# dvl-tum/e-osvos

Measured on AMD Instinct MI355X. Metric: finetune_iters_per_sec, higher is better.
Workload: dtype f32 (f16x3 split); 1 GPU; e-OSVOS-50 fine-tune iteration (BASELINE configs[1]): DeepLabV3+-ResNet50, batch 3, 480x854, BCE, per-neuron-lr SGD; one (sequence, object) per rank; batch=3, height=480, width=854, parallelism=replicas x1

## Files before the change

### e-osvos_amd/_ffi.py

```python
import ctypes
import os

_HERE = os.path.dirname(os.path.abspath(__file__))
LIB_PATH = os.environ.get('EOSVOS_LIB') or os.path.join(_HERE, 'libeosvos.so')

c_float_p = ctypes.c_void_p
_E = ctypes.c_void_p


class View(ctypes.Structure):
    _fields_ = [('p', ctypes.c_void_p), ('ld', ctypes.c_int), ('key', ctypes.c_void_p), ('ldkey', ctypes.c_int)]


class ConvViews(ctypes.Structure):
    _fields_ = ([(n, ctypes.c_int) for n in ('algo', 'B', 'H', 'W', 'Cin', 'Cout', 'k', 'stride', 'dil', 'pad')] +
                [('w_oihw', ctypes.c_void_p), ('scale', ctypes.c_void_p), ('bias', ctypes.c_void_p), ('passes', ctypes.c_int),
                 ('x', View), ('y', View), ('res', View), ('relu', ctypes.c_int), ('y_m8', ctypes.c_void_p),
                 ('g', View), ('gx', View), ('add', View), ('accum', ctypes.c_int), ('mask_c0', ctypes.c_int),
                 ('gx_m8', ctypes.c_void_p), ('dw_oihw', ctypes.c_void_p),
                 ('slot_bits', ctypes.c_uint * 2), ('slot_valid', ctypes.c_int * 2),
                 ('src_slot_bits', ctypes.c_uint * 2), ('src_slot_valid', ctypes.c_int * 2), ('fwd_slices', ctypes.c_int)])


VIEWS_FWD, VIEWS_DGRAD, VIEWS_WGRAD = 1, 2, 4
# ... 59 lines not shown
    'eosvos_bce': (ctypes.c_int, [_E, c_float_p, c_float_p, ctypes.c_int64, c_float_p, c_float_p]),
    'eosvos_backward_step': (ctypes.c_int, [_E, ctypes.c_int]),
    'eosvos_finetune_step': (ctypes.c_int, [_E, c_float_p, c_float_p, ctypes.c_int, ctypes.c_int,
                                            ctypes.POINTER(ctypes.c_float)]),
    'eosvos_keep_grads': (ctypes.c_int, [_E, ctypes.c_int]),
    'eosvos_get_grads': (ctypes.c_int, [_E, c_float_p]),
    'eosvos_infer': (ctypes.c_int, [_E, c_float_p, ctypes.c_int, c_float_p]),
    'eosvos_infer_view': (ctypes.c_int, [_E, c_float_p, ctypes.c_int, ctypes.c_int]),
    'eosvos_tta_accumulate': (ctypes.c_int, [_E, ctypes.c_int, ctypes.c_int, ctypes.c_int, ctypes.c_int, ctypes.c_float, ctypes.c_int,
                                             c_float_p, ctypes.c_int, ctypes.c_int]),
    'eosvos_resize_frames': (ctypes.c_int, [_E, c_float_p] + [ctypes.c_int] * 6 + [c_float_p]),
    'eosvos_merge_labels': (ctypes.c_int, [_E, c_float_p, ctypes.c_int, ctypes.c_int64, ctypes.c_void_p]),
    'eosvos_meta_task_begin': (ctypes.c_int, [_E]),
    'eosvos_meta_grad': (ctypes.c_int, [_E, c_float_p, c_float_p, ctypes.c_int, c_float_p,
                                        ctypes.POINTER(ctypes.c_float)]),
    'eosvos_meta_grad_ex': (ctypes.c_int, [_E, c_float_p, c_float_p, ctypes.c_int, c_float_p,
                                           ctypes.POINTER(ctypes.c_float), ctypes.c_float, ctypes.c_int]),
    'eosvos_radam_step': (ctypes.c_int, [_E, c_float_p, c_float_p, c_float_p, c_float_p, ctypes.c_int64,
                                         ctypes.c_float, ctypes.c_float, ctypes.c_float, ctypes.c_float,
                                         ctypes.c_float, ctypes.c_int, ctypes.c_float, ctypes.c_float]),
    'eosvos_clamp': (ctypes.c_int, [_E, c_float_p, ctypes.c_int64, ctypes.c_float, ctypes.c_float]),
    'eosvos_outer_step': (ctypes.c_int, [_E, c_float_p, c_float_p, c_float_p, c_float_p, ctypes.c_int64, ctypes.c_int, ctypes.c_int,
                                         ctypes.c_float, ctypes.c_float, ctypes.c_float, ctypes.c_float, ctypes.c_float,
                                         ctypes.c_float, ctypes.c_float, ctypes.c_float, ctypes.c_float, ctypes.c_float,
                                         ctypes.c_int, ctypes.c_int64, ctypes.c_int64]),
    'eosvos_alias_state': (ctypes.c_int, [_E, _E]),
    'eosvos_unalias_state': (ctypes.c_int, [_E]),
    'eosvos_set_trainable_from': (ctypes.c_int, [_E, ctypes.c_int]),
    'eosvos_comm_unique_id': (ctypes.c_int, [ctypes.c_void_p]),
    'eosvos_comm_init_rank': (ctypes.c_int, [ctypes.POINTER(ctypes.c_void_p), ctypes.c_int, ctypes.c_void_p, ctypes.c_int, ctypes.c_int]),
    'eosvos_comm_destroy': (ctypes.c_int, [ctypes.c_void_p]),
    'eosvos_allreduce_sum': (ctypes.c_int, [_E, c_float_p, ctypes.c_int64, ctypes.c_void_p]),
    'eosvos_time_hot_kernel': (ctypes.c_int, [_E, ctypes.c_int, ctypes.c_int, ctypes.POINTER(ctypes.c_float),
                                              ctypes.POINTER(ctypes.c_double)]),
    'eosvos_bench_conv': (ctypes.c_int, [_E, ctypes.c_int, ctypes.c_int, ctypes.c_int, ctypes.c_int,
                                         ctypes.POINTER(ctypes.c_float), ctypes.POINTER(ctypes.c_double)]),
    'eosvos_mfma_probe': (ctypes.c_int, [_E, ctypes.c_int, ctypes.POINTER(ctypes.c_float),
                                         ctypes.POINTER(ctypes.c_double)]),
    'eosvos_profile_launches': (ctypes.c_int, [_E, ctypes.c_int]),
    'eosvos_profile_read': (ctypes.c_int, [_E, ctypes.c_int, ctypes.c_char_p, ctypes.POINTER(ctypes.c_int64),
                                           ctypes.POINTER(ctypes.c_double), ctypes.POINTER(ctypes.c_double),
                                           ctypes.POINTER(ctypes.c_int)]),
    'eosvos_debug_tensor': (ctypes.c_int, [_E, ctypes.c_char_p, ctypes.POINTER(ctypes.c_void_p),
                                           ctypes.POINTER(ctypes.c_int64)]),
    'eosvos_test_conv': (ctypes.c_int, [_E, c_float_p, c_float_p, c_float_p, c_float_p, c_float_p,
                                        ctypes.c_int] + [ctypes.c_int] * 9 + [c_float_p]),
    'eosvos_test_conv_bwd': (ctypes.c_int, [_E, c_float_p, c_float_p, c_float_p] + [ctypes.c_int] * 9 +
                             [c_float_p, c_float_p]),
    'eosvos_test_conv_algo': (ctypes.c_int, [_E, ctypes.c_int, c_float_p, c_float_p, c_float_p, c_float_p, c_float_p,
                                             ctypes.c_int] + [ctypes.c_int] * 9 + [c_float_p]),
    'eosvos_test_conv_bwd_algo': (ctypes.c_int, [_E, ctypes.c_int, c_float_p, c_float_p, c_float_p, c_float_p, ctypes.c_void_p] +
                                  [ctypes.c_int] * 9 + [c_float_p, c_float_p]),
    'eosvos_test_conv_views': (ctypes.c_int, [_E, ctypes.POINTER(ConvViews)]),
    'eosvos_test_aspp_dgrad': (ctypes.c_int, [_E, ctypes.c_int, c_float_p, ctypes.c_void_p, c_float_p, ctypes.c_int,
                                              ctypes.POINTER(ctypes.c_int), ctypes.POINTER(ctypes.c_uint),
                                              ctypes.POINTER(ctypes.c_int)]),
    'eosvos_test_groupnorm': (ctypes.c_int, [_E, ctypes.c_int, c_float_p, ctypes.c_int, c_float_p, ctypes.c_int, c_float_p,
                                             c_float_p, c_float_p, ctypes.c_int, ctypes.c_int, ctypes.c_int, ctypes.c_int,
                                             ctypes.c_int, ctypes.c_float, c_float_p, ctypes.c_int, c_float_p, ctypes.c_void_p,
                                             ctypes.c_int]),
    'eosvos_test_maxpool': (ctypes.c_int, [_E, c_float_p] + [ctypes.c_int] * 4 + [c_float_p, ctypes.c_void_p, c_float_p, c_float_p]),
    'eosvos_test_resize': (ctypes.c_int, [_E] + [ctypes.c_int] * 7 + [c_float_p, ctypes.c_int] * 4 + [ctypes.c_void_p, ctypes.c_int]),
    'eosvos_test_aspp_pool': (ctypes.c_int, [_E] + [ctypes.c_int] * 4 + [c_float_p] * 4 + [ctypes.c_int] + [c_float_p] * 3 +
                              [ctypes.c_int, ctypes.c_void_p, ctypes.c_int, c_float_p, ctypes.c_int] + [c_float_p] * 4 +
                              [ctypes.c_int]),
    'eosvos_test_head': (ctypes.c_int, [_E, c_float_p, c_float_p, c_float_p, ctypes.c_int64, ctypes.c_int] + [c_float_p] * 4),
    'eosvos_test_wgrad_presplit': (ctypes.c_int, [c_float_p] * 8 + [ctypes.c_int] * 15 + [ctypes.c_void_p]),
}

_lib = None


class EosvosError(RuntimeError):
    pass


def load():
    global _lib
    if _lib is not None:
        return _lib
    if not os.path.exists(LIB_PATH):
        raise EosvosError(
            f'{LIB_PATH} is missing: build it with `python -c "import __graft_entry__ as g; g.build()"` '
            '(hipcc --offload-arch=gfx950).  There is no CPU fallback.')
    lib = ctypes.CDLL(LIB_PATH)
    for name, (res, args) in _SIGNATURES.items():
        fn = getattr(lib, name)
        fn.restype = res
        fn.argtypes = args
    _lib = lib
    return lib


def exported_symbols():
    return sorted(_SIGNATURES)


def check(rc):
    if rc != 0:
        raise EosvosError(load().eosvos_last_error().decode() or f'eosvos call failed ({rc})')
```

### e-osvos_amd/csrc/engine.cpp

```cpp
#include <dlfcn.h>
#include <hip/hip_runtime.h>
#include <math.h>
#include <stdio.h>
#include <stdlib.h>
#include <string.h>

#include <algorithm>
#include <cmath>
#include <functional>
#include <map>
#include <set>
#include <string>
#include <vector>

#include "../../include/eosvos.h"
#include "kernels.h"

using namespace eosvos;

static thread_local std::string g_err;
static int fail(const std::string& m) {
  g_err = m;
  return 1;
}
// ... 3086 lines not shown
  launch_oihw_to_ohwi(w_oihw, t->Wp, Cout, Cin, k * k, t->s);
  if (scale) {
    HIPOK(hipMemcpyAsync(t->na, scale, (size_t)Cout * 4, hipMemcpyDeviceToDevice, t->s));
    HIPOK(hipMemcpyAsync(t->nb, bias, (size_t)Cout * 4, hipMemcpyDeviceToDevice, t->s));
  }
  if (res && wino_on(t, 0, B, conv_out(H, k, stride, dil, pad), conv_out(W, k, stride, dil, pad)))
    return fail("the Winograd output transform has no residual input (the network never needs one)");
  conv_fwd(t, 0, x, Cin, H, W, y, Cout, B, res, Cout, relu != 0);
  HIPOK(hipStreamSynchronize(t->s));
  HIPOK(hipGetLastError());
  return 0;
}
int eosvos_test_conv_bwd_algo(eosvos_engine* e, int algo, const float* x, const float* w_oihw, const float* g,
                              const float* scale, const uint8_t* m8, int B, int H, int W, int Cin, int Cout, int k, int stride,
                              int dil, int pad, float* dx, float* dw_oihw) {
  ModeScope mode_scope(e);
  if (!e || !x || !w_oihw || !g || !dx || !dw_oihw) return fail("null argument");
  if (Cin % 4 || Cout % 4) return fail("channels must be multiples of 4");
  if (algo < EOSVOS_ALGO_AUTO || algo > EOSVOS_ALGO_WINO_F4) return fail("unknown conv algorithm");
  ScratchEngine se(e, algo, B, H, W, Cin, Cout, k, stride, dil, pad, scale != nullptr);
  if (!se.ok) return fail("scratch engine: shape not eligible for the requested algorithm, or out of memory");
  eosvos_engine* t = &se.t;
  const int T = k * k;
  amax_new_phase(t, 0);
  amax_new_phase(t, 1);
  launch_oihw_to_ohwi(w_oihw, t->Wp, Cout, Cin, T, t->s);
  if (scale) HIPOK(hipMemcpyAsync(t->na, scale, (size_t)Cout * 4, hipMemcpyDeviceToDevice, t->s));
  conv_wgrad(t, 0, g, Cout, x, Cin, H, W, B);
  if (m8) t->mask8[x] = const_cast<uint8_t*>(m8);
  if (conv_dgrad(t, 0, g, Cout, H, W, dx, Cin, B, false, m8 ? x : nullptr, 0)) return 1;
  float* dw = t->falloc((int64_t)Cout * Cin * T);
  if (!dw) return fail("hipMalloc dw");
  const int64_t n = (int64_t)Cout * Cin * T;
  launch_sgd_update(dw, t->ws_wg, t->upd_splits[0], n, scale ? t->na : nullptr, nullptr, nullptr, dw, (int64_t)T * Cin, n, t->s);
  launch_ohwi_to_oihw(dw, dw_oihw, Cout, Cin, T, 1.f, 0, t->s);
  HIPOK(hipStreamSynchronize(t->s));
  HIPOK(hipGetLastError());
  return 0;
}
int eosvos_test_conv(eosvos_engine* e, const float* x, const float* w_oihw, const float* scale, const float* bias,
                     const float* res, int relu, int B, int H, int W, int Cin, int Cout, int k, int stride, int dil,
                     int pad, float* y) {
  ModeScope mode_scope(e);
  return eosvos_test_conv_algo(e, EOSVOS_ALGO_DIRECT, x, w_oihw, scale, bias, res, relu, B, H, W, Cin, Cout, k, stride, dil, pad, y);
}
int eosvos_test_conv_bwd(eosvos_engine* e, const float* x, const float* w_oihw, const float* g, int B, int H, int W,
                         int Cin, int Cout, int k, int stride, int dil, int pad, float* dx, float* dw_oihw) {
  ModeScope mode_scope(e);
  return eosvos_test_conv_bwd_algo(e, EOSVOS_ALGO_DIRECT, x, w_oihw, g, nullptr, nullptr, B, H, W, Cin, Cout, k, stride, dil, pad, dx,
                                   dw_oihw);
}

namespace {
int read_tslot(eosvos_engine* t, int phase, const float* key, unsigned* bits, int* valid) {
  *bits = 0; *valid = 0;
  if (!h3_mode() || !t->amax) return 0;
  auto it = t->treg[phase].find(key);
  if (it == t->treg[phase].end()) return 0;
  unsigned w[AMAX_SUB];
  HIPOK(hipMemcpy2D(w, sizeof(unsigned), t->amax + amax_tcol(t, phase, it->second.idx), (size_t)AMAX_ROW * sizeof(unsigned),
                    sizeof(unsigned), AMAX_SUB, hipMemcpyDeviceToHost));
  for (int i = 0; i < AMAX_SUB; ++i) *bits = w[i] > *bits ? w[i] : *bits;
  *valid = it->second.valid ? 1 : 0;
  return 0;
}
int seed_tslot(eosvos_engine* t, int phase, const float* key, long rows, int C) {
  if (!h3_mode()) return 0;
  if (amax_init(t)) return fail("absmax arena");
  unsigned* sl = tslot(t, phase, key);
  if (!sl) return fail("no absmax slot left for the source tensor");
  launch_absmax(key, rows, C, C, sl, t->s);
  tmark_valid(t, phase, key);
  return 0;
}
bool view_ok(const eosvos_view& v, int C) {
  if (!v.p || v.ld < C || (v.ld & 3)) return false;
  if (!v.key) return true;
  const long off = v.p - v.key;
  return v.ldkey == v.ld && off >= 0 && !(off & 3) && off + C <= v.ldkey;
}
}

int eosvos_test_conv_views(eosvos_engine* e, eosvos_conv_views* v) {
  ModeScope mode_scope(e);
  if (!e || !v || !v->w_oihw) return fail("null argument");
  const int B = v->B, H = v->H, W = v->W, Cin = v->Cin, Cout = v->Cout, k = v->k;
  if (B < 1 || H < 1 || W < 1 || Cin < 4 || Cout < 4 || (Cin % 4) || (Cout % 4)) return fail("bad geometry (channels must be multiples of 4)");
  if (v->algo < EOSVOS_ALGO_AUTO || v->algo > EOSVOS_ALGO_WINO_F4) return fail("unknown conv algorithm");
  const bool fwd = v->passes & EOSVOS_VIEWS_FWD, dg = v->passes & EOSVOS_VIEWS_DGRAD, wg = v->passes & EOSVOS_VIEWS_WGRAD;
  if (!fwd && !dg && !wg) return fail("no pass selected");
  if (fwd && (v->scale == nullptr) != (v->bias == nullptr)) return fail("scale and bias go together (folded norm)");
  if (fwd && (!view_ok(v->x, Cin) || !view_ok(v->y, Cout) || (v->res.p && !view_ok(v->res, Cout)))) return fail("bad forward view");
  const int nsl = v->fwd_slices > 1 ? v->fwd_slices : 1;
  if (nsl > 1) {
    if (!fwd || dg || wg || v->res.p || !v->x.key || !v->y.key) return fail("fwd_slices: forward only, keyed x and y, no residual");
    if ((v->x.p - v->x.key) + (long)nsl * Cin > v->x.ldkey || (v->y.p - v->y.key) + (long)nsl * Cout > v->y.ldkey) return fail("fwd_slices: past the tensor");
  }
  if ((dg || wg) && !view_ok(v->g, Cout)) return fail("bad gradient view");
  if (dg && (!view_ok(v->gx, Cin) || (v->add.p && !view_ok(v->add, Cin)) || v->mask_c0 < 0 || (v->mask_c0 & 3))) return fail("bad data-gradient view");
  if (wg && (!view_ok(v->x, Cin) || !v->dw_oihw)) return fail("bad weight-gradient view");
  ScratchEngine se(e, v->algo, B, H, W, Cin, Cout, k, v->stride, v->dil, v->pad, v->scale != nullptr);
  if (!se.ok) return fail("scratch engine: shape not eligible for the requested algorithm, or out of memory");
  eosvos_engine* t = &se.t;
  const int T = k * k;
  const int Ho = conv_out(H, k, v->stride, v->dil, v->pad), Wo = conv_out(W, k, v->stride, v->dil, v->pad);
  const long Pin = (long)B * H * W, Pout = (long)B * Ho * Wo;
// ... 231 lines not shown
```

### e-osvos_amd/csrc/kernels.h

```cpp
#pragma once
#include <hip/hip_runtime.h>
#include <stdint.h>

namespace eosvos {
#define AMAX_SUB 32
#define AMAX_ROW 2048
#if defined(__HIPCC__)
__device__ __forceinline__ unsigned amax_f1(float x) {
  const unsigned a = __float_as_uint(x) & 0x7fffffffu;
  return a < 0x7f800000u ? a : 0u;
}
__device__ __forceinline__ unsigned amax_f4(unsigned m, const float4& v) {
  const unsigned a = amax_f1(v.x), b = amax_f1(v.y), c = amax_f1(v.z), d = amax_f1(v.w);
  const unsigned ab = a > b ? a : b, cd = c > d ? c : d;
  const unsigned q = ab > cd ? ab : cd;
  return m > q ? m : q;
}
__device__ __forceinline__ uint8_t relu_bits(const float4& v) {
  return (uint8_t)((v.x > 0.f ? 1 : 0) | (v.y > 0.f ? 2 : 0) | (v.z > 0.f ? 4 : 0) | (v.w > 0.f ? 8 : 0));
}
__device__ __forceinline__ void relu_mask8(float4& v, unsigned bits) {
  v.x = (bits & 1u) ? v.x : 0.f; v.y = (bits & 2u) ? v.y : 0.f; v.z = (bits & 4u) ? v.z : 0.f; v.w = (bits & 8u) ? v.w : 0.f;
}
__device__ __forceinline__ void amax_block_commit(unsigned m, unsigned* slot) {
// ... 147 lines not shown
  int B, Ho, Wo, ldg, Cout;
  int Hi, Wi, ldx, Cin;
  int KH, KW, stride, pad, dil;
  int splits;
  long g_tap_stride, x_tap_stride;
  const unsigned* amax_g;
  const unsigned* amax_x;
  float* scn_g; float* scn_x;
  int margin_g, margin_x;
};
void launch_wgrad(const WgradArgs& a, hipStream_t s);
int wgrad_pick_splits(int P, int Cout, int Cin, int T, int wg_budget = 0, int mode = -1);
int wgrad_group_tile(int channels);
void launch_wgrad_group(const WgradArgs* dev_tab, const int* dev_map, int nwg, int bm, int bn, double flops, hipStream_t s);
struct WgradPArgs {
  const unsigned char* g2;
  const unsigned char* x2;
  float* ws;
  int B, Ho, Wo, ldg, Cout;
  int Hi, Wi, ldx, Cin;
  int KH, KW, stride, pad, dil;
  int splits;
  int groups;
  long g_tap_stride, x_tap_stride;
  const unsigned char* zero;
  const float* scp_g; const float* scp_x;
  const unsigned* slot_g; const unsigned* slot_x;
  float* scn_g; float* scn_x;
  int margin_g, margin_x;
  const float* g; const float* x;
};
#define PAIR_HEADROOM 10
bool wgrad_p_supported(const WgradPArgs& a);
int wgrad_p_tiles(const WgradPArgs& a);
void launch_wgrad_p(const WgradPArgs& a, hipStream_t s);
int wgrad_p_pick_splits(int P, int Cout, int Cin, int T, int wg_budget);
int wgrad_p_resident(int wg_budget);
void launch_wgrad_p_group(const WgradPArgs* dev_tab, const int* dev_map, int nwg, double flops, hipStream_t s);
void launch_pair_split(const float* x, void* out, long rows, int C, int ld, const unsigned* slot, int margin, float* sc, hipStream_t s);
int conv_wg_budget_of(int requested);
int conv_clamp_wg_budget(int n);
void launch_wino_input(int tm, const float* x, int ldx, int C, int B, int H, int W, int th, int tw, int dil, long prow, float* V,
                       hipStream_t s, unsigned* amax = nullptr);
void launch_wino_grad(int tm, const float* g, int ldg, int C, int B, int H, int W, int th, int tw, int dil, long prow, float* M,
                      hipStream_t s, unsigned* amax = nullptr);
void launch_wino_weight(int tm, const float* w, int Cout, int Cin, const float* rowscale, float* U, float* Us, hipStream_t s,
                        unsigned* amax_u = nullptr, unsigned* amax_us = nullptr);
void launch_wino_output(int tm, const float* M, long prow, int C, int B, int H, int W, int th, int tw, int dil, const float* scale,
                        const float* bias, int relu, float* y, int ldy, hipStream_t s, unsigned* amax = nullptr,
                        uint8_t* mask8_out = nullptr, int ldm8 = 0);
void launch_wino_wgrad_finish(int tm, const float* ws, int splits, int Cout, int Cin, float* dst, hipStream_t s);
void launch_wino_dgrad_output(int tm, const float* dV, long prow, int C, int B, int H, int W, int th, int tw, int dil,
                              const uint8_t* mask8, int ldm8, int mask_c0, int accum, float* gx, int ldgx, hipStream_t s,
                              unsigned* amax = nullptr);

void launch_nchw_to_nhwc_pad(const float* src, float* dst, int B, int C, int H, int W, int pad,
                             hipStream_t s, unsigned* amax = nullptr, int mirror = 0);
void launch_fill(float* p, int64_t n, float v, hipStream_t s);
void launch_oihw_to_ohwi(const float* src, float* dst, int O, int I, int T, hipStream_t s);
void launch_ohwi_to_oihw(const float* src, float* dst, int O, int I, int T, float alpha, int add,
                         hipStream_t s);
void launch_fold_norm(const float* gamma, const float* beta, const float* mean, const float* var,
                      float eps, float* a, float* b, int64_t n, hipStream_t s);

void launch_stem_fwd(const float* xpad, const float* w , const float* a,
                     const float* b, float* y, int B, int H, int W, int Ho, int Wo, hipStream_t s);
void launch_stem_wgrad(const float* xpad, const float* g, float* ws , int B,
                       int H, int W, int Ho, int Wo, int chunks, hipStream_t s);
int stem_wgrad_chunks(int B, int Ho, int Wo);
void launch_stem_fwd_h3(const float* xpad, const float* w , const float* a, const float* b, float* y, int B,
                        int H, int W, int Ho, int Wo, const unsigned* amax_x, hipStream_t s);
void launch_stem_wgrad_h3(const float* xpad, const float* g, float* ws , int B, int H, int W, int Ho,
                          int Wo, int chunks, const unsigned* amax_g, const unsigned* amax_x, hipStream_t s);

void launch_maxpool_fwd(const float* x, float* y, uint8_t* idx, int B, int H, int W, int C, int Ho,
                        int Wo, hipStream_t s, unsigned* amax = nullptr);
void launch_maxpool_bwd(const float* gy, const uint8_t* idx, float* gx, int B, int H,
                        int W, int C, int Ho, int Wo, hipStream_t s, unsigned* amax = nullptr);

struct ResizeTab {
  int in, out;
  const int* i0;
  const int* i1;
  const float* lam;
  const int* lo;
  const int* hi;
};
void launch_resize_fwd(const float* x, int ldx, float* y, int ldy, int B, int C, ResizeTab th,
                       ResizeTab tw, hipStream_t s);
void launch_resize_bwd(const float* gy, int ldgy, float* gx, int ldgx, const uint8_t* m8, int ldm8,
                       int B, int C, ResizeTab th, ResizeTab tw, hipStream_t s, unsigned* amax = nullptr);

void launch_colsum(const float* x, int ldx, float* out , int B, int P, int C, float alpha,
                   float* scratch, hipStream_t s);
void launch_gemv_fwd(const float* W, const float* v, const float* a, const float* b, float* y, int B,
                     int N, int K, hipStream_t s);
void launch_gemv_bwd(const float* W, const float* v, const float* gp, const float* a, float* gv,
                     float* dW, int B, int N, int K, hipStream_t s);
void launch_bcast_pixels(const float* v , float* y, int ldy, int B, int P, int C, float alpha,
                         hipStream_t s, uint8_t* mask8_out = nullptr, int ldm8 = 0);

void launch_last_fwd(const float* x, const float* w, const float* bias, float* y, int64_t P, int C,
                     hipStream_t s);
void launch_last_bwd(const float* x, const float* w, const float* g, float* gx, float* ws_dw,
                     int64_t P, int C, int chunks, hipStream_t s);
int last_bwd_chunks(int64_t P);

// ... 106 lines not shown
```

### e-osvos_amd/csrc/misc_kernels.hip

```cpp
#include <cassert>

#include "kernels.h"

namespace eosvos {

__device__ __forceinline__ float wave_sum(float v) {
#pragma unroll
  for (int o = 32; o > 0; o >>= 1) v += __shfl_xor(v, o, 64);
  return v;
}
__device__ __forceinline__ float block_sum_256(float v, float* sh ) {
  v = wave_sum(v);
  const int w = threadIdx.x >> 6;
  __syncthreads();
  if ((threadIdx.x & 63) == 0) sh[w] = v;
  __syncthreads();
  return sh[0] + sh[1] + sh[2] + sh[3];
}
static inline int grid_for(long n, int per_block, int cap = 4096) {
  long b = (n + per_block - 1) / per_block;
  if (b < 1) b = 1;
  if (b > cap) b = cap;
  return (int)b;
}
// ... 2058 lines not shown
        const int tx = blk.tx + dl;
        if ((unsigned)tx >= (unsigned)tw) continue;
        const long tile = ((((long)b * dil + sy) * dil + sx) * th + ty) * tw + tx;
#pragma unroll
        for (int ii = 0; ii < 2; ++ii) {
          const int i = dk < 0 ? 3 : (dk > 0 ? 0 : 1 + ii);
          if (dk != 0 && ii == 1) continue;
          const int r = dk < 0 ? 0 : (dk > 0 ? 1 : ii);
#pragma unroll
          for (int jj = 0; jj < 2; ++jj) {
            const int j = dl < 0 ? 3 : (dl > 0 ? 0 : 1 + jj);
            if (dl != 0 && jj == 1) continue;
            const int q = dl < 0 ? 0 : (dl > 0 ? 1 : jj);
            float4 sum = zero4();
#pragma unroll
            for (int a = 0; a < 4; ++a) {
              if (Mt::BT[a][i] == 0.f) continue;
#pragma unroll
              for (int bb = 0; bb < 4; ++bb) {
                if (Mt::BT[bb][j] == 0.f) continue;
                const float4 v = *reinterpret_cast<const float4*>(dV + ((long)(a * 4 + bb) * prow + tile) * C + c4 * 4);
                const float wgt = Mt::BT[a][i] * Mt::BT[bb][j];
                sum.x += wgt * v.x; sum.y += wgt * v.y; sum.z += wgt * v.z; sum.w += wgt * v.w;
              }
            }
            acc[r][q].x += sum.x; acc[r][q].y += sum.y; acc[r][q].z += sum.z; acc[r][q].w += sum.w;
          }
        }
      }
    }
#pragma unroll
    for (int r = 0; r < 2; ++r) {
      const int yy = sy + dil * (2 * blk.ty + r);
      if (yy >= H) continue;
#pragma unroll
      for (int q = 0; q < 2; ++q) {
        const int xx = sx + dil * (2 * blk.tx + q);
        if (xx >= W) continue;
        const long pix = ((long)b * H + yy) * W + xx;
        float4 v = acc[r][q];
        if (accum) {
          const float4 o = *reinterpret_cast<const float4*>(gx + pix * ldgx + c4 * 4);
          v.x += o.x; v.y += o.y; v.z += o.z; v.w += o.w;
        }
        if (mask8 && c4 * 4 >= mask_c0) relu_mask8(v, mask8[pix * ldm8 + c4]);
        am = amax_f4(am, v);
        *reinterpret_cast<float4*>(gx + pix * ldgx + c4 * 4) = v;
      }
    }
  }
  if (amax) amax_block_commit(am, amax);
}

#define WINO_LAUNCH(kernel, grid, s, ...)                                                              \
  do {                                                                                                 \
    assert(tm == 2 || tm == 4);                                                                        \
    if (tm == 4) hipLaunchKernelGGL(kernel<4>, dim3(grid), dim3(256), 0, s, __VA_ARGS__);              \
    else hipLaunchKernelGGL(kernel<2>, dim3(grid), dim3(256), 0, s, __VA_ARGS__);                      \
  } while (0)
void launch_wino_input(int tm, const float* x, int ldx, int C, int B, int H, int W, int th, int tw, int dil, long prow, float* V,
                       hipStream_t s, unsigned* amax) {
  const long n = (long)B * dil * dil * th * tw * (C / 4);
  WINO_LAUNCH(wino_input_kernel, grid_for(n, 256, 8192), s, x, ldx, C, B, H, W, th, tw, dil, prow, V, amax);
}
void launch_wino_grad(int tm, const float* g, int ldg, int C, int B, int H, int W, int th, int tw, int dil, long prow, float* M,
                      hipStream_t s, unsigned* amax) {
  const long n = (long)B * dil * dil * th * tw * (C / 4);
  WINO_LAUNCH(wino_grad_kernel, grid_for(n, 256, 8192), s, g, ldg, C, B, H, W, th, tw, dil, prow, M, amax);
}
void launch_wino_weight(int tm, const float* w, int Cout, int Cin, const float* rowscale, float* U, float* Us, hipStream_t s,
                        unsigned* amax_u, unsigned* amax_us) {
  const long n = (long)Cout * (Cin / 4);
  WINO_LAUNCH(wino_weight_kernel, grid_for(n, 256), s, w, Cout, Cin, rowscale, U, Us, amax_u, amax_us);
}
void launch_wino_output(int tm, const float* M, long prow, int C, int B, int H, int W, int th, int tw, int dil, const float* scale,
                        const float* bias, int relu, float* y, int ldy, hipStream_t s, unsigned* amax, uint8_t* mask8_out, int ldm8) {
  const long n = (long)B * dil * dil * th * tw * (C / 4);
  WINO_LAUNCH(wino_output_kernel, grid_for(n, 256, 8192), s, M, prow, C, B, H, W, th, tw, dil, scale, bias, relu, y, ldy, amax,
              relu ? mask8_out : nullptr, ldm8);
}
void launch_wino_wgrad_finish(int tm, const float* ws, int splits, int Cout, int Cin, float* dst, hipStream_t s) {
  const long n = (long)Cout * (Cin / (tm == 4 ? wino_finish_cin_per_thread<4> : wino_finish_cin_per_thread<2>));
  WINO_LAUNCH(wino_wgrad_finish_kernel, grid_for(n, 256), s, ws, splits, Cout, Cin, dst);
}
void launch_wino_dgrad_output(int tm, const float* dV, long prow, int C, int B, int H, int W, int th, int tw, int dil,
                              const uint8_t* mask8, int ldm8, int mask_c0, int accum, float* gx, int ldgx, hipStream_t s,
                              unsigned* amax) {
  const long n = (long)B * dil * dil * th * tw * (C / 4);
  WINO_LAUNCH(wino_dgrad_output_kernel, grid_for(n, 256, 8192), s, dV, prow, C, B, H, W, th, tw, dil, mask8, ldm8, mask_c0, accum,
              gx, ldgx, amax);
}
#undef WINO_LAUNCH
}
```

### e-osvos_amd/engine.py

```python
import ctypes

import torch

from . import _ffi
from .topology import ARCH_ID, norm_layers, trainable


def _ptr(t):
    return ctypes.c_void_p(t.data_ptr())


def _optr(t):
    return _ptr(t) if t is not None else None


def _relu_bits(t):
    if t is None:
        return None
    m = (t > 0).to(torch.uint8).reshape(*t.shape[:-1], -1, 4)
    return (m[..., 0] | (m[..., 1] << 1) | (m[..., 2] << 2) | (m[..., 3] << 3)).contiguous()


def _ld(t):
    if t is None:
# ... 662 lines not shown
        _ffi.check(self.lib.eosvos_mfma_probe(self.h, iters, ctypes.byref(ms), ctypes.byref(fl)))
        return fl.value / (ms.value * 1e-3) / 1e12

    def debug_tensor(self, name):
        ptr = ctypes.c_void_p()
        dims = (ctypes.c_int64 * 4)()
        _ffi.check(self.lib.eosvos_debug_tensor(self.h, name.encode(), ctypes.byref(ptr), dims))
        b, h, w, c = [int(d) for d in dims]
        n = b * h * w * c
        out = torch.empty(n, device=self.device)
        self.synchronize()
        import ctypes as _c
        hip = _c.CDLL('libamdhip64.so')
        rc = hip.hipMemcpy(_c.c_void_p(out.data_ptr()), ptr, _c.c_size_t(n * 4), 3)
        if rc != 0:
            raise _ffi.EosvosError(f'hipMemcpy failed ({rc})')
        return out.view(b, h, w, c).permute(0, 3, 1, 2).contiguous()

    def test_conv(self, x_nhwc, w_oihw, scale, bias, res, relu, stride, dil, pad):
        B, H, W, Cin = x_nhwc.shape
        Cout, _, k, _ = w_oihw.shape
        Ho = (H + 2 * pad - dil * (k - 1) - 1) // stride + 1
        Wo = (W + 2 * pad - dil * (k - 1) - 1) // stride + 1
        y = torch.empty(B, Ho, Wo, Cout, device=self.device)
        p = lambda t: _ptr(t) if t is not None else None
        _ffi.check(self.lib.eosvos_test_conv(self.h, _ptr(x_nhwc), _ptr(w_oihw), p(scale), p(bias), p(res),
                                             int(relu), B, H, W, Cin, Cout, k, stride, dil, pad, _ptr(y)))
        return y

    ALGOS = {'auto': 0, 'direct': 1, 'wino_f2': 2, 'wino_f4': 3}

    def test_conv_algo(self, algo, x_nhwc, w_oihw, scale, bias, res, relu, stride, dil, pad):
        B, H, W, Cin = x_nhwc.shape
        Cout, _, k, _ = w_oihw.shape
        Ho = (H + 2 * pad - dil * (k - 1) - 1) // stride + 1
        Wo = (W + 2 * pad - dil * (k - 1) - 1) // stride + 1
        y = torch.empty(B, Ho, Wo, Cout, device=self.device)
        p = lambda t: _ptr(t) if t is not None else None
        _ffi.check(self.lib.eosvos_test_conv_algo(self.h, self.ALGOS[algo], _ptr(x_nhwc), _ptr(w_oihw), p(scale), p(bias),
                                                  p(res), int(relu), B, H, W, Cin, Cout, k, stride, dil, pad, _ptr(y)))
        return y

    def test_conv_bwd_algo(self, algo, x_nhwc, w_oihw, g_nhwc, stride, dil, pad, scale=None, mask=None):
        B, H, W, Cin = x_nhwc.shape
        Cout, _, k, _ = w_oihw.shape
        dx = torch.empty_like(x_nhwc)
        dw = torch.empty_like(w_oihw)
        m8 = _relu_bits(mask)
        _ffi.check(self.lib.eosvos_test_conv_bwd_algo(self.h, self.ALGOS[algo], _ptr(x_nhwc), _ptr(w_oihw), _ptr(g_nhwc),
                                                      _optr(scale), _optr(m8), B, H, W, Cin, Cout, k, stride, dil, pad, _ptr(dx),
                                                      _ptr(dw)))
        return dx, dw

    def test_conv_bwd(self, x_nhwc, w_oihw, g_nhwc, stride, dil, pad):
        B, H, W, Cin = x_nhwc.shape
        Cout, _, k, _ = w_oihw.shape
        dx = torch.empty_like(x_nhwc)
        dw = torch.empty_like(w_oihw)
        _ffi.check(self.lib.eosvos_test_conv_bwd(self.h, _ptr(x_nhwc), _ptr(w_oihw), _ptr(g_nhwc), B, H, W, Cin,
                                                 Cout, k, stride, dil, pad, _ptr(dx), _ptr(dw)))
        return dx, dw

    @staticmethod
    def _view(t, C, shape):
        v = _ffi.View()
        if t is None:
            return v
        view, base = t if isinstance(t, tuple) else (t, None)
        B, h, w = shape
        ld = view.stride(2)
        assert view.dtype == torch.float32 and tuple(view.shape) == (B, h, w, C), (tuple(view.shape), (B, h, w, C))
        assert view.stride() == (h * w * ld, w * ld, ld, 1) and ld >= C and ld % 4 == 0, view.stride()
        v.p, v.ld = view.data_ptr(), ld
        if base is None:
            assert view.is_contiguous() or view._base is not None, 'a strided view needs its base tensor'
            if view._base is not None:
                b0 = view._base
                off = (view.data_ptr() - b0.data_ptr()) // 4
                assert 0 <= off and off + (B * h * w - 1) * ld + C <= b0.numel(), 'view outside its storage'
        else:
            assert base.dtype == torch.float32 and base.is_contiguous() and tuple(base.shape) == (B, h, w, ld), tuple(base.shape)
            off = (view.data_ptr() - base.data_ptr()) // 4
            assert 0 <= off <= ld - C and off % 4 == 0, off
            v.key, v.ldkey = base.data_ptr(), ld
        return v

    def test_conv_views(self, algo, w_oihw, stride, dil, pad, shape, scale=None, bias=None, x=None, y=None, res=None, relu=False,
                        y_m8=None, g=None, gx=None, add=None, accum=False, mask_c0=0, gx_m8=None, want_dw=False, fwd_slices=1):
        B, H, W = shape
        Cout, Cin, k, _ = w_oihw.shape
        Ho = (H + 2 * pad - dil * (k - 1) - 1) // stride + 1
        Wo = (W + 2 * pad - dil * (k - 1) - 1) // stride + 1
        a = _ffi.ConvViews()
        a.algo, a.B, a.H, a.W, a.Cin, a.Cout, a.k, a.stride, a.dil, a.pad = self.ALGOS[algo], B, H, W, Cin, Cout, k, stride, dil, pad
        assert w_oihw.is_contiguous() and w_oihw.dtype == torch.float32
        a.w_oihw = w_oihw.data_ptr()
        for name, t in (('scale', scale), ('bias', bias)):
            if t is not None:
                assert t.is_contiguous() and t.dtype == torch.float32 and t.numel() == Cout
                setattr(a, name, t.data_ptr())
        a.passes = (_ffi.VIEWS_FWD if y is not None else 0) | (_ffi.VIEWS_DGRAD if gx is not None else 0) | (_ffi.VIEWS_WGRAD if want_dw else 0)
        a.x, a.y, a.res = self._view(x, Cin, (B, H, W)), self._view(y, Cout, (B, Ho, Wo)), self._view(res, Cout, (B, Ho, Wo))
        a.g, a.gx, a.add = self._view(g, Cout, (B, Ho, Wo)), self._view(gx, Cin, (B, H, W)), self._view(add, Cin, (B, H, W))
        a.relu, a.accum, a.mask_c0, a.fwd_slices = int(relu), int(accum), int(mask_c0), int(fwd_slices)
        if fwd_slices > 1:
            for vw, C in ((a.x, Cin), (a.y, Cout)):
# ... 106 lines not shown
```

### include/eosvos.h

```cpp
#ifndef EOSVOS_H
#define EOSVOS_H

#include <stddef.h>
#include <stdint.h>

#ifdef __cplusplus
extern "C" {
#endif

typedef struct eosvos_engine eosvos_engine;

#define EOSVOS_ARCH_RESNET50 50
#define EOSVOS_ARCH_RESNET101 101
#define EOSVOS_ARCH_V3_RESNET50 1050
#define EOSVOS_ARCH_V3_RESNET101 1101
#define EOSVOS_NORM_BN_FROZEN 0
#define EOSVOS_NORM_GN16 1

const char* eosvos_version(void);
const char* eosvos_last_error(void);

#define EOSVOS_MATRIX_F32 0
#define EOSVOS_MATRIX_BF16X6 1
#define EOSVOS_MATRIX_F16X3 2
// ... 108 lines not shown
                     float* flat_meta_grad, float* meta_loss_host);
#define EOSVOS_META_INIT_GRAD 1
#define EOSVOS_META_NEW_SEGMENT 2
int eosvos_meta_grad_ex(eosvos_engine* e, const float* images, const float* masks, int batch,
                        float* flat_meta_grad, float* meta_loss_host, float weight, int flags);

int eosvos_radam_step(eosvos_engine* e, float* param, const float* grad, float* exp_avg,
                      float* exp_avg_sq, int64_t n, float lr, float weight_decay, float beta1,
                      float beta2, float eps, int step, float grad_scale, float grad_clip);
int eosvos_clamp(eosvos_engine* e, float* param, int64_t n, float lo, float hi);
int eosvos_outer_step(eosvos_engine* e, float* state, float* grad, float* exp_avg, float* exp_avg_sq, int64_t n_lr,
                      int learn_model_init, int step, float lr_lr, float init_lr, float weight_decay, float beta1, float beta2,
                      float eps, float grad_scale, float grad_clip, float lr_lo, float lr_hi, int use_log,
                      int64_t frozen_lr, int64_t frozen_param);
int eosvos_alias_state(eosvos_engine* e, eosvos_engine* src);
int eosvos_unalias_state(eosvos_engine* e);

int eosvos_set_trainable_from(eosvos_engine* e, int conv_idx);

typedef struct { char internal[128]; } eosvos_rccl_id;
int eosvos_comm_unique_id(eosvos_rccl_id* id);
int eosvos_comm_init_rank(void** comm, int world_size, const eosvos_rccl_id* id, int rank, int device_id);
int eosvos_comm_destroy(void* comm);
int eosvos_allreduce_sum(eosvos_engine* e, float* flat, int64_t n, void* comm);

int eosvos_time_hot_kernel(eosvos_engine* e, int batch, int reps, float* ms_host,
                           double* flops_host);
int eosvos_bench_conv(eosvos_engine* e, int conv_idx, int kind, int batch, int reps, float* ms_host,
                      double* flops_host);
int eosvos_mfma_probe(eosvos_engine* e, int iters, float* ms_host, double* flops_host);
int eosvos_profile_launches(eosvos_engine* e, int on);
int eosvos_profile_read(eosvos_engine* e, int max_kernels, char* names, int64_t* counts, double* ms_host,
                        double* flops_host, int* n_out_host);
int eosvos_debug_tensor(eosvos_engine* e, const char* name, float** ptr_out, int64_t* dims4_out);
int eosvos_test_conv(eosvos_engine* e, const float* x_nhwc, const float* w_oihw,
                     const float* scale, const float* bias, const float* res_nhwc, int relu,
                     int B, int H, int W, int Cin, int Cout, int k, int stride, int dil, int pad,
                     float* y_nhwc);
#define EOSVOS_ALGO_AUTO 0
#define EOSVOS_ALGO_DIRECT 1
#define EOSVOS_ALGO_WINO_F2 2
#define EOSVOS_ALGO_WINO_F4 3
int eosvos_test_conv_algo(eosvos_engine* e, int algo, const float* x_nhwc, const float* w_oihw,
                          const float* scale, const float* bias, const float* res_nhwc, int relu,
                          int B, int H, int W, int Cin, int Cout, int k, int stride, int dil, int pad,
                          float* y_nhwc);
int eosvos_test_conv_bwd_algo(eosvos_engine* e, int algo, const float* x_nhwc, const float* w_oihw,
                              const float* g_nhwc, const float* scale, const uint8_t* m8, int B, int H, int W,
                              int Cin, int Cout, int k, int stride, int dil, int pad, float* dx_nhwc,
                              float* dw_oihw);
int eosvos_test_conv_bwd(eosvos_engine* e, const float* x_nhwc, const float* w_oihw,
                         const float* g_nhwc, int B, int H, int W, int Cin, int Cout, int k,
                         int stride, int dil, int pad, float* dx_nhwc, float* dw_oihw);

typedef struct eosvos_view {
  float* p;
  int ld;
  float* key;
  int ldkey;
} eosvos_view;
#define EOSVOS_VIEWS_FWD 1
#define EOSVOS_VIEWS_DGRAD 2
#define EOSVOS_VIEWS_WGRAD 4
typedef struct eosvos_conv_views {
  int algo, B, H, W, Cin, Cout, k, stride, dil, pad;
  const float* w_oihw;
  const float* scale;
  const float* bias;
  int passes;
  eosvos_view x, y, res;
  int relu;
  uint8_t* y_m8;
  eosvos_view g, gx, add;
  int accum, mask_c0;
  const uint8_t* gx_m8;
  float* dw_oihw;
  unsigned slot_bits[2];
  int slot_valid[2];
  unsigned src_slot_bits[2];
  int src_slot_valid[2];
  int fwd_slices;
} eosvos_conv_views;
int eosvos_test_conv_views(eosvos_engine* e, eosvos_conv_views* v);
int eosvos_test_aspp_dgrad(eosvos_engine* e, int batch, const float* g_cat, const uint8_t* l4_m8, float* g_l4_inout,
                           int force_fallback, int* merged_ran, unsigned* slot_bits, int* slot_valid);

int eosvos_test_groupnorm(eosvos_engine* e, int bwd, float* z, int ldz, const float* g, int ldg, const float* gamma,
                          const float* beta, const float* res, int ldres, int relu, int B, int P, int C, float eps, float* y,
                          int ldy, float* stats, uint8_t* m8, int ldm8);
int eosvos_test_maxpool(eosvos_engine* e, const float* x, int B, int H, int W, int C, float* y, uint8_t* idx, const float* gy,
                        float* gx);
int eosvos_test_resize(eosvos_engine* e, int align_corners, int hin, int win, int hout, int wout, int B, int C, const float* x,
                       int ldx, float* y, int ldy, const float* gy, int ldgy, float* gx, int ldgx, const uint8_t* m8, int ldm8);
int eosvos_test_aspp_pool(eosvos_engine* e, int B, int P, int K, int N, const float* w, const float* a, const float* bias,
                          const float* x, int ldx, float* v, float* pool, float* y, int ldy, uint8_t* m8, int ldm8,
                          const float* gy, int ldgy, float* gpool, float* gv, float* dw, float* gx, int ldgx);
int eosvos_test_head(eosvos_engine* e, const float* x, const float* w, const float* bias, int64_t P, int C, float* y,
                     const float* g, float* gx, float* dw);

int eosvos_test_wgrad_presplit(const float* g, const float* x, float* ws, void* g2, void* x2, unsigned* amax, float* sc,
                               const void* zero, int B, int Ho, int Wo, int Cout, int Hi, int Wi, int Cin, int k, int stride,
                               int pad, int dil, int splits, int groups, int margin, int which, void* stream);

#ifdef __cplusplus
}
#endif
// ... 2 lines not shown
```

Baseline: 114.5 finetune_iters/s.

## Share Winograd F4 dgrad output-transform partials between neighbour tiles via LDS

Adds an LDS-based Winograd F(4,3) dgrad output kernel. Each thread handles one tile and channel quad within a 4x4 tile block, computes its own stage-1 transform once, and exchanges edge rows and columns with neighbouring tiles through shared memory, instead of re-reading and re-transforming neighbour dV tiles from global memory. The kernel becomes the default for tm=4, dil=1. Tiles on a block boundary still fall back to global loads. The cost is extra registers (a 6x6 float4 array per thread), several barriers, and a new test entry point to compare the two forms.

New measurement: 115.0 finetune_iters/s, median of 6. No clear change (+0.5%).

```diff
diff --git a/e-osvos_amd/_ffi.py b/e-osvos_amd/_ffi.py
--- a/e-osvos_amd/_ffi.py
+++ b/e-osvos_amd/_ffi.py
@@ -135,6 +135,9 @@
     'eosvos_test_conv_bwd_algo': (ctypes.c_int, [_E, ctypes.c_int, c_float_p, c_float_p, c_float_p, c_float_p, ctypes.c_void_p] +
                                   [ctypes.c_int] * 9 + [c_float_p, c_float_p]),
     'eosvos_test_conv_views': (ctypes.c_int, [_E, ctypes.POINTER(ConvViews)]),
+    'eosvos_test_wino_dgrad_output': (ctypes.c_int, [_E, ctypes.c_int, c_float_p] + [ctypes.c_int] * 4 + [ctypes.c_void_p,
+                                                     ctypes.c_int, ctypes.c_int, c_float_p, ctypes.c_int,
+                                                     ctypes.POINTER(ctypes.c_uint)]),
     'eosvos_test_aspp_dgrad': (ctypes.c_int, [_E, ctypes.c_int, c_float_p, ctypes.c_void_p, c_float_p, ctypes.c_int,
                                               ctypes.POINTER(ctypes.c_int), ctypes.POINTER(ctypes.c_uint),
                                               ctypes.POINTER(ctypes.c_int)]),
diff --git a/e-osvos_amd/csrc/engine.cpp b/e-osvos_amd/csrc/engine.cpp
--- a/e-osvos_amd/csrc/engine.cpp
+++ b/e-osvos_amd/csrc/engine.cpp
@@ -3162,6 +3162,41 @@
 }
 
 namespace {
+struct TestAmaxArena {
+  unsigned* d = nullptr;
+  TestAmaxArena() {
+    if (hipMalloc(&d, (size_t)AMAX_SUB * AMAX_ROW * sizeof(unsigned)) != hipSuccess) d = nullptr;
+    if (d) (void)hipMemset(d, 0, (size_t)AMAX_SUB * AMAX_ROW * sizeof(unsigned));
+  }
+  ~TestAmaxArena() { if (d) (void)hipFree(d); }
+  unsigned* slot(int s) const { return d + s; }
+  int read(int s, unsigned* bits) const {
+    unsigned w[AMAX_SUB];
+    HIPOK(hipMemcpy2D(w, sizeof(unsigned), d + s, (size_t)AMAX_ROW * sizeof(unsigned), sizeof(unsigned), AMAX_SUB, hipMemcpyDeviceToHost));
+    *bits = 0;
+    for (int i = 0; i < AMAX_SUB; ++i) *bits = w[i] > *bits ? w[i] : *bits;
+    return 0;
+  }
+};
+}
+int eosvos_test_wino_dgrad_output(eosvos_engine* e, int form, const float* dV, int B, int H, int W, int C, const uint8_t* m8,
+                                  int mask_c0, int accum, float* gx, int ldgx, unsigned* amax_bits) {
+  if (!e || !dV || !gx || !amax_bits) return fail("null argument");
+  if (form < 0 || form > 1) return fail("form: 0 gather, 1 LDS");
+  if (B < 1 || H < 1 || W < 1 || C < 4 || (C & 3) || ldgx < C || (ldgx & 3) || mask_c0 < 0 || (mask_c0 & 3)) return fail("bad geometry");
+  if (form == 1 && !wino_dgrad_output_lds_ok(4, 1, C)) return fail("the LDS form does not take this shape");
+  const int th = (H + 3) / 4, tw = (W + 3) / 4;
+  const long ntile = (long)B * th * tw;
+  TestAmaxArena am;
+  if (!am.d) return fail("hipMalloc absmax arena");
+  launch_wino_dgrad_output(4, dV, ntile, C, B, H, W, th, tw, 1, m8, ldgx / 4, mask_c0, accum ? 1 : 0, gx, ldgx, e->s, am.slot(0),
+                           form == 0);
+  HIPOK(hipStreamSynchronize(e->s));
+  HIPOK(hipGetLastError());
+  return am.read(0, amax_bits);
+}
+
+namespace {
 int read_tslot(eosvos_engine* t, int phase, const float* key, unsigned* bits, int* valid) {
   *bits = 0; *valid = 0;
   if (!h3_mode() || !t->amax) return 0;
diff --git a/e-osvos_amd/csrc/kernels.h b/e-osvos_amd/csrc/kernels.h
--- a/e-osvos_amd/csrc/kernels.h
+++ b/e-osvos_amd/csrc/kernels.h
@@ -223,7 +223,8 @@
 void launch_wino_wgrad_finish(int tm, const float* ws, int splits, int Cout, int Cin, float* dst, hipStream_t s);
 void launch_wino_dgrad_output(int tm, const float* dV, long prow, int C, int B, int H, int W, int th, int tw, int dil,
                               const uint8_t* mask8, int ldm8, int mask_c0, int accum, float* gx, int ldgx, hipStream_t s,
-                              unsigned* amax = nullptr);
+                              unsigned* amax = nullptr, bool gather = false);
+bool wino_dgrad_output_lds_ok(int tm, int dil, int C);
 
 void launch_nchw_to_nhwc_pad(const float* src, float* dst, int B, int C, int H, int W, int pad,
                              hipStream_t s, unsigned* amax = nullptr, int mirror = 0);
diff --git a/e-osvos_amd/csrc/misc_kernels.hip b/e-osvos_amd/csrc/misc_kernels.hip
--- a/e-osvos_amd/csrc/misc_kernels.hip
+++ b/e-osvos_amd/csrc/misc_kernels.hip
@@ -2134,6 +2134,212 @@
   if (amax) amax_block_commit(am, amax);
 }
 
+constexpr int WDG_BX = 4, WDG_BY = 4, WDG_CQ = 16;
+static_assert(WDG_BX * WDG_BY * WDG_CQ == 256, "one thread per (tile position, channel quad) of the block");
+template <int DK, int DL>
+__device__ __forceinline__ void wino4_dg_stage1_global(const float* __restrict__ dV, long prow, long tile, int C, int c4,
+                                                       float4 (&t)[4][6]) {
+  using Mt = WinoMat<4>;
+  constexpr int TM = 4, NP = 6, ni = DK == 0 ? TM : 1;
+#pragma unroll
+  for (int ii = 0; ii < TM; ++ii)
+#pragma unroll
+    for (int bb = 0; bb < NP; ++bb) t[ii][bb] = zero4();
+#pragma unroll
+  for (int a = 0; a < NP; ++a) {
+    if (DK < 0 && a != NP - 1) continue;
+    if (DK > 0 && a != 0) continue;
+#pragma unroll
+    for (int bb = 0; bb < NP; ++bb) {
+      if (DL < 0 && bb != NP - 1) continue;
+      if (DL > 0 && bb != 0) continue;
+      const float4 v = *reinterpret_cast<const float4*>(dV + ((long)(a * NP + bb) * prow + tile) * C + c4 * 4);
+#pragma unroll
+      for (int ii = 0; ii < TM; ++ii) {
+        if (ii >= ni) continue;
+        const int i = DK < 0 ? NP - 1 : (DK > 0 ? 0 : 1 + ii);
+        if (Mt::BT[a][i] != 0.f) fma4(t[ii][bb], Mt::BT[a][i], v);
+      }
+    }
+  }
+}
+template <int DK, int DL>
+__device__ __forceinline__ void wino4_dg_stage2(float4 (&acc)[4][4], const float4 (&t)[4][6]) {
+  using Mt = WinoMat<4>;
+  constexpr int TM = 4, NP = 6, ni = DK == 0 ? TM : 1, nj = DL == 0 ? TM : 1;
+#pragma unroll
+  for (int ii = 0; ii < TM; ++ii) {
+    if (ii >= ni) continue;
+    const int r = DK < 0 ? 0 : (DK > 0 ? TM - 1 : ii);
+#pragma unroll
+    for (int jj = 0; jj < TM; ++jj) {
+      if (jj >= nj) continue;
+      const int j = DL < 0 ? NP - 1 : (DL > 0 ? 0 : 1 + jj);
+      const int q = DL < 0 ? 0 : (DL > 0 ? TM - 1 : jj);
+#pragma unroll
+      for (int bb = 0; bb < NP; ++bb) {
+        if (DL < 0 && bb != NP - 1) continue;
+        if (DL > 0 && bb != 0) continue;
+        if (Mt::BT[bb][j] != 0.f) fma4(acc[r][q], Mt::BT[bb][j], t[ii][bb]);
+      }
+    }
+  }
+}
+__global__ __launch_bounds__(256) void wino_dgrad_output_lds_kernel(const float* __restrict__ dV, long prow, int C, int B, int H,
+                                                                     int W, int th, int tw, const uint8_t* __restrict__ mask8,
+                                                                     int ldm8, int mask_c0, int accum, float* __restrict__ gx,
+                                                                     int ldgx, unsigned* __restrict__ amax) {
+  using Mt = WinoMat<4>;
+  constexpr int TM = 4, NP = 6;
+  __shared__ float4 xch[NP][256];
+  const int C4 = C >> 2;
+  const int nch = (C4 + WDG_CQ - 1) / WDG_CQ, nbx = (tw + WDG_BX - 1) / WDG_BX, nby = (th + WDG_BY - 1) / WDG_BY;
+  const int tid = threadIdx.x, cq = tid & (WDG_CQ - 1), bx = (tid / WDG_CQ) % WDG_BX, by = tid / (WDG_CQ * WDG_BX);
+  int bid = blockIdx.x;
+  const int c4 = (bid % nch) * WDG_CQ + cq; bid /= nch;
+  const int tx = (bid % nbx) * WDG_BX + bx; bid /= nbx;
+  const int ty = (bid % nby) * WDG_BY + by;
+  const int b = bid / nby;
+  const bool on = c4 < C4 && tx < tw && ty < th;
+  const long tile = ((long)b * th + ty) * tw + tx;
+  const bool up = on && ty > 0, down = on && ty + 1 < th, left = on && tx > 0, right = on && tx + 1 < tw;
+  const bool lup = by > 0, ldown = by + 1 < WDG_BY, lleft = bx > 0, lright = bx + 1 < WDG_BX;
+  constexpr int SY = WDG_CQ * WDG_BX, SX = WDG_CQ;
+  float4 T[NP][NP];
+  if (on) {
+#pragma unroll
+    for (int a = 0; a < NP; ++a)
+#pragma unroll
+      for (int bb = 0; bb < NP; ++bb)
+        T[a][bb] = *reinterpret_cast<const float4*>(dV + ((long)(a * NP + bb) * prow + tile) * C + c4 * 4);
+#pragma unroll
+    for (int bb = 0; bb < NP; ++bb) {
+      float4 c[NP];
+#pragma unroll
+      for (int i = 0; i < NP; ++i) {
+        c[i] = zero4();
+#pragma unroll
+        for (int a = 0; a < NP; ++a)
+          if (Mt::BT[a][i] != 0.f) fma4(c[i], Mt::BT[a][i], T[a][bb]);
+      }
+#pragma unroll
+      for (int i = 0; i < NP; ++i) T[i][bb] = c[i];
+    }
+  } else {
+#pragma unroll
+    for (int a = 0; a < NP; ++a)
+#pragma unroll
+      for (int bb = 0; bb < NP; ++bb) T[a][bb] = zero4();
+  }
+  float4 acc[TM][TM];
+#pragma unroll
+  for (int r = 0; r < TM; ++r)
+#pragma unroll
+    for (int q = 0; q < TM; ++q) acc[r][q] = zero4();
+  float4 t[TM][NP];
+#pragma unroll
+  for (int bb = 0; bb < NP; ++bb) xch[bb][tid] = T[NP - 1][bb];
+  __syncthreads();
+  if (up) {
+    if (left) {
+      if (lup && lleft) t[0][NP - 1] = xch[NP - 1][tid - SY - SX];
+      else wino4_dg_stage1_global<-1, -1>(dV, prow, tile - tw - 1, C, c4, t);
+      wino4_dg_stage2<-1, -1>(acc, t);
+    }
+    if (lup) {
+#pragma unroll
+      for (int bb = 0; bb < NP; ++bb) t[0][bb] = xch[bb][tid - SY];
+    } else {
+      wino4_dg_stage1_global<-1, 0>(dV, prow, tile - tw, C, c4, t);
+    }
+    wino4_dg_stage2<-1, 0>(acc, t);
+    if (right) {
+      if (lup && lright) t[0][0] = xch[0][tid - SY + SX];
+      else wino4_dg_stage1_global<-1, 1>(dV, prow, tile - tw + 1, C, c4, t);
+      wino4_dg_stage2<-1, 1>(acc, t);
+    }
+  }
+  __syncthreads();
+#pragma unroll
+  for (int ii = 0; ii < TM; ++ii) xch[ii][tid] = T[1 + ii][NP - 1];
+  __syncthreads();
+  if (left) {
+    if (lleft) {
+#pragma unroll
+      for (int ii = 0; ii < TM; ++ii) t[ii][NP - 1] = xch[ii][tid - SX];
+    } else {
+      wino4_dg_stage1_global<0, -1>(dV, prow, tile - 1, C, c4, t);
+    }
+    wino4_dg_stage2<0, -1>(acc, t);
+  }
+  if (on) {
+#pragma unroll
+    for (int ii = 0; ii < TM; ++ii)
+#pragma unroll
+      for (int bb = 0; bb < NP; ++bb) t[ii][bb] = T[1 + ii][bb];
+    wino4_dg_stage2<0, 0>(acc, t);
+  }
+  __syncthreads();
+#pragma unroll
+  for (int ii = 0; ii < TM; ++ii) xch[ii][tid] = T[1 + ii][0];
+  __syncthreads();
+  if (right) {
+    if (lright) {
+#pragma unroll
+      for (int ii = 0; ii < TM; ++ii) t[ii][0] = xch[ii][tid + SX];
+    } else {
+      wino4_dg_stage1_global<0, 1>(dV, prow, tile + 1, C, c4, t);
+    }
+    wino4_dg_stage2<0, 1>(acc, t);
+  }
+  __syncthreads();
+#pragma unroll
+  for (int bb = 0; bb < NP; ++bb) xch[bb][tid] = T[0][bb];
+  __syncthreads();
+  if (down) {
+    if (left) {
+      if (ldown && lleft) t[0][NP - 1] = xch[NP - 1][tid + SY - SX];
+      else wino4_dg_stage1_global<1, -1>(dV, prow, tile + tw - 1, C, c4, t);
+      wino4_dg_stage2<1, -1>(acc, t);
+    }
+    if (ldown) {
+#pragma unroll
+      for (int bb = 0; bb < NP; ++bb) t[0][bb] = xch[bb][tid + SY];
+    } else {
+      wino4_dg_stage1_global<1, 0>(dV, prow, tile + tw, C, c4, t);
+    }
+    wino4_dg_stage2<1, 0>(acc, t);
+    if (right) {
+      if (ldown && lright) t[0][0] = xch[0][tid + SY + SX];
+      else wino4_dg_stage1_global<1, 1>(dV, prow, tile + tw + 1, C, c4, t);
+      wino4_dg_stage2<1, 1>(acc, t);
+    }
+  }
+  unsigned am = 0;
+  if (on) {
+#pragma unroll
+    for (int r = 0; r < TM; ++r) {
+      const int yy = TM * ty + r;
+#pragma unroll
+      for (int q = 0; q < TM; ++q) {
+        const int xx = TM * tx + q;
+        if (yy < H && xx < W) {
+          const long pix = ((long)b * H + yy) * W + xx;
+          float4 v = acc[r][q];
+          if (accum) {
+            const float4 o = *reinterpret_cast<const float4*>(gx + pix * ldgx + c4 * 4);
+            v.x += o.x; v.y += o.y; v.z += o.z; v.w += o.w;
+          }
+          if (mask8 && c4 * 4 >= mask_c0) relu_mask8(v, mask8[pix * ldm8 + c4]);
+          am = amax_f4(am, v);
+          *reinterpret_cast<float4*>(gx + pix * ldgx + c4 * 4) = v;
+        }
+      }
+    }
+  }
+  if (amax) amax_block_commit(am, amax);
+}
+
 #define WINO_LAUNCH(kernel, grid, s, ...)                                                              \
   do {                                                                                                 \
     assert(tm == 2 || tm == 4);                                                                        \
@@ -2165,9 +2371,17 @@
   const long n = (long)Cout * (Cin / (tm == 4 ? wino_finish_cin_per_thread<4> : wino_finish_cin_per_thread<2>));
   WINO_LAUNCH(wino_wgrad_finish_kernel, grid_for(n, 256), s, ws, splits, Cout, Cin, dst);
 }
+bool wino_dgrad_output_lds_ok(int tm, int dil, int C) { return tm == 4 && dil == 1 && (C & 3) == 0; }
 void launch_wino_dgrad_output(int tm, const float* dV, long prow, int C, int B, int H, int W, int th, int tw, int dil,
                               const uint8_t* mask8, int ldm8, int mask_c0, int accum, float* gx, int ldgx, hipStream_t s,
-                              unsigned* amax) {
+                              unsigned* amax, bool gather) {
+  if (!gather && wino_dgrad_output_lds_ok(tm, dil, C)) {
+    const long nwg = (long)B * ((th + WDG_BY - 1) / WDG_BY) * ((tw + WDG_BX - 1) / WDG_BX) * ((C / 4 + WDG_CQ - 1) / WDG_CQ);
+    assert(nwg > 0 && nwg < (1L << 31));
+    hipLaunchKernelGGL(wino_dgrad_output_lds_kernel, dim3((unsigned)nwg), dim3(256), 0, s, dV, prow, C, B, H, W, th, tw, mask8,
+                       ldm8, mask_c0, accum, gx, ldgx, amax);
+    return;
+  }
   const long n = (long)B * dil * dil * th * tw * (C / 4);
   WINO_LAUNCH(wino_dgrad_output_kernel, grid_for(n, 256, 8192), s, dV, prow, C, B, H, W, th, tw, dil, mask8, ldm8, mask_c0, accum,
               gx, ldgx, amax);
diff --git a/e-osvos_amd/engine.py b/e-osvos_amd/engine.py
--- a/e-osvos_amd/engine.py
+++ b/e-osvos_amd/engine.py
@@ -738,6 +738,16 @@
                                                       _ptr(dw)))
         return dx, dw
 
+    def test_wino_dgrad_output(self, form, dV, gx, C, m8=None, mask_c0=0, accum=False):
+        B, H, W, ldgx = gx.shape
+        nt = B * ((H + 3) // 4) * ((W + 3) // 4)
+        assert dV.is_contiguous() and tuple(dV.shape) == (36, nt, C) and gx.is_contiguous()
+        assert m8 is None or (m8.dtype == torch.uint8 and m8.is_contiguous() and tuple(m8.shape) == (B, H, W, ldgx // 4))
+        bits = ctypes.c_uint(0)
+        _ffi.check(self.lib.eosvos_test_wino_dgrad_output(self.h, form, _ptr(dV), B, H, W, C, _optr(m8), mask_c0, int(accum),
+                                                          _ptr(gx), ldgx, ctypes.byref(bits)))
+        return bits.value
+
     def test_conv_bwd(self, x_nhwc, w_oihw, g_nhwc, stride, dil, pad):
         B, H, W, Cin = x_nhwc.shape
         Cout, _, k, _ = w_oihw.shape
diff --git a/include/eosvos.h b/include/eosvos.h
--- a/include/eosvos.h
+++ b/include/eosvos.h
@@ -184,6 +184,8 @@
 int eosvos_test_conv_bwd(eosvos_engine* e, const float* x_nhwc, const float* w_oihw,
                          const float* g_nhwc, int B, int H, int W, int Cin, int Cout, int k,
                          int stride, int dil, int pad, float* dx_nhwc, float* dw_oihw);
+int eosvos_test_wino_dgrad_output(eosvos_engine* e, int form, const float* dV, int B, int H, int W, int C, const uint8_t* m8,
+                                  int mask_c0, int accum, float* gx, int ldgx, unsigned* amax_bits);
 
 typedef struct eosvos_view {
   float* p;
```
